# zhihu/rucene

Measured on AMD Instinct MI355X. Metric: queries/sec + postings decoded/sec, BM25 10M-doc synthetic, higher is better.
Workload: dtype u32 decode + f32 BM25

## Files before the change

rucene_amd/csrc/kernels/search_term.hpp:

```cpp
#pragma once
#include "search.hpp"

namespace rgpu {

#ifdef RGPU_EXP_COUNT
__device__ unsigned long long g_term_dbg[4];
#endif

#ifndef RGPU_TERM_PRUNE
#define RGPU_TERM_PRUNE 1
#endif
#ifndef RGPU_TERM_ORDER
#define RGPU_TERM_ORDER 1
#endif
#ifndef RGPU_TERM_EXCHANGE
#define RGPU_TERM_EXCHANGE 2
#endif
#ifndef RGPU_TERM_EXCHANGE_MAX_ITEMS
#define RGPU_TERM_EXCHANGE_MAX_ITEMS 16
#endif
#ifndef RGPU_TERM_WAIT
#define RGPU_TERM_WAIT 0
#endif
#ifndef RGPU_TERM_WAIT_POLLS
// ... 42 lines not shown
  const uint64_t v = __hip_atomic_load(g.keys + (k - 1), __ATOMIC_RELAXED, __HIP_MEMORY_SCOPE_WORKGROUP);
  return ((uint64_t)(uint32_t)readfirstlane((int)(uint32_t)(v >> 32)) << 32) | (uint32_t)readfirstlane((int)(uint32_t)v);
}
#ifndef RGPU_TERM_RANK_MERGE
#define RGPU_TERM_RANK_MERGE 0
#endif
#ifndef RGPU_TERM_RANK_MERGE_MAX
#define RGPU_TERM_RANK_MERGE_MAX 16
#endif
#ifndef RGPU_TERM_LEVEL_CUT
#define RGPU_TERM_LEVEL_CUT 1
#endif
#ifndef RGPU_TERM_LEVEL_CUT_MIN
#define RGPU_TERM_LEVEL_CUT_MIN 16
#endif
#ifdef RGPU_TERM_TRACE
#define TERM_LK_PARAM , uint32_t (&lk)[4]
#define TERM_LK_NOW(v) const uint64_t v = (uint64_t)clock64()
#define TERM_LK_ADD(i, since) lk[i] += (uint32_t)((uint64_t)clock64() - (since))
#define TERM_LK_COUNT(i, n) lk[i] += (uint32_t)(n)
#define TERM_LK_DECL uint32_t lk[4] = {0, 0, 0, 0}
#define TERM_LK_PASS , lk
#else
#define TERM_LK_PARAM
#define TERM_LK_DECL do {} while (0)
#define TERM_LK_PASS
#define TERM_LK_NOW(v) do {} while (0)
#define TERM_LK_ADD(i, since) do {} while (0)
#define TERM_LK_COUNT(i, n) do {} while (0)
#endif
static_assert(RGPU_TERM_RANK_MERGE_MAX >= 3 && RGPU_TERM_RANK_MERGE_MAX <= 64 && 8 * RGPU_TERM_RANK_MERGE_MAX <= TERM_BLOCK_SLAB,
              "the candidates of a rank merge fit one register and the staging slab");
template <bool WIDE>
__device__ __forceinline__ void group_offer2(const GroupList& g, uint64_t key0, uint64_t key1, uint64_t& tau, int k, int lane,
                                             uint64_t floor, uint8_t* slab TERM_LK_PARAM) {
#if RGPU_TERM_LEVEL_CUT
  if (!WIDE && __popcll(__ballot(key0 > tau)) + __popcll(__ballot(key1 > tau)) > (k > RGPU_TERM_LEVEL_CUT_MIN ? k : RGPU_TERM_LEVEL_CUT_MIN)) {
    uint32_t level = 0xffffffffu;
    for (int have = 0; have < k;) {
      const uint32_t h0 = (uint32_t)(key0 >> 32), h1 = (uint32_t)(key1 >> 32);
      const uint32_t b0 = h0 < level ? h0 : 0u, b1 = h1 < level ? h1 : 0u;
      const uint32_t t = wave_reduce_max_u32(b0 > b1 ? b0 : b1);
      if (t == 0u) { level = 0u; break; }
      have += __popcll(__ballot(h0 == t)) + __popcll(__ballot(h1 == t));
      level = t;
    }
    key0 = (uint32_t)(key0 >> 32) >= level ? key0 : 0ull;
    key1 = (uint32_t)(key1 >> 32) >= level ? key1 : 0ull;
  }
#endif
  TERM_LK_NOW(lk_t0);
  TERM_LK_COUNT(2, 1);
  group_lock(g.lock, lane);
  TERM_LK_ADD(0, lk_t0);
  TERM_LK_NOW(lk_t1);
  WaveTopK top;
  top.a = g.keys[lane];
  if (WIDE) top.b = g.keys[64 + lane];
  const uint64_t kth = topk_threshold<WIDE>(top, k);
  tau = kth > floor ? kth : floor;
#if RGPU_TERM_RANK_MERGE
  const uint64_t m0 = __ballot(key0 > tau), m1 = __ballot(key1 > tau);
  const int n0 = __popcll(m0), n = n0 + __popcll(m1);
  TERM_LK_COUNT(3, n);
  if (!WIDE && n > 2 && n <= RGPU_TERM_RANK_MERGE_MAX) {
    uint64_t* stage = reinterpret_cast<uint64_t*>(slab);
    int ln = lane;
    asm volatile("" : "+v"(ln));
    if ((m0 >> ln) & 1ull) stage[mbcnt(m0)] = key0;
    if ((m1 >> ln) & 1ull) stage[n0 + mbcnt(m1)] = key1;
    wave_sync();
    const uint64_t c = ln < n ? stage[ln] : 0ull;
    wave_sync();
    const uint64_t L = top.a;
    int shift = 0;
    for (int i = 0; i < n; ++i) {
      const uint64_t x = readlane64(c, i);
      const bool above = L > x;
      const int at = __popcll(__ballot(above)) + __popcll(__ballot(c > x));
      shift += above ? 0 : 1;
      if (ln == i && at < 64) g.keys[at] = c;
    }
    if (ln + shift < 64) g.keys[ln + shift] = L;
// ... 569 lines not shown
```

rucene_amd/csrc/kernels/search_term_query.hpp:

```cpp
#pragma once
#include "search_term.hpp"

namespace rgpu {

#ifndef RGPU_TERMQ_CAP
#define RGPU_TERMQ_CAP 256
#endif
constexpr int TQ_CAP = RGPU_TERMQ_CAP;
constexpr int TQ_CHUNK_UNROLL = 4;
#ifndef RGPU_TERMQ_STEP_CHUNKS
#define RGPU_TERMQ_STEP_CHUNKS 2
#endif
constexpr int TQ_STEP_CHUNKS = RGPU_TERMQ_STEP_CHUNKS;
#ifndef RGPU_TERMQ_FAST_WAVES
#define RGPU_TERMQ_FAST_WAVES RGPU_TERM_FAST_WAVES
#endif
static_assert(TQ_CAP >= 64 && TQ_CAP <= 65536, "queue positions are u16 and a chunk must fit an empty queue");

__device__ __forceinline__ uint32_t term_thr_of(uint64_t t, int32_t lo) {
  const uint32_t thi = (uint32_t)(t >> 32);
  if (!(thi & 0x80000000u)) return 0u;
  const uint32_t bits = thi & 0x7fffffffu;
  return key_doc(t) <= lo + 1 ? bits + 1u : bits;
}
__device__ __forceinline__ uint32_t term_bound_of(const float* cache, uint64_t w) {
  const uint32_t fmax = (uint32_t)w & 15u;
  uint32_t bb = 0u;
#pragma unroll
  for (int f = 1; f <= SCORE_TABLE_FREQS; ++f) {
    const uint32_t r = (uint32_t)(w >> (4 + 6 * (f - 1))) & 63u;
    const uint32_t sc = __float_as_uint(table_score(cache, r, (uint32_t)f));
    bb = ((uint32_t)f <= fmax && sc > bb) ? sc : bb;
  }
  return fmax > (uint32_t)SCORE_TABLE_FREQS ? 0xffffffffu : bb;
}

#ifdef RGPU_TERM_TRACE
struct TermQueryTraceRec {
  unsigned long long t0, t1;
  int32_t q, nblocks, rounds, entries, unpacked, offers, entered;
  unsigned int d[7];
  unsigned int waves, wave0_cycles;
  unsigned int cyc[8][3];
  unsigned int pad[16];
};
static_assert(sizeof(TermQueryTraceRec) == 3 * sizeof(TermTraceRec), "a workgroup's record takes three slots of g_term_trace");
#define TQ_TR(slot, dep) do { asm volatile("" :: "v"(dep)); tq_d[slot] = (unsigned int)((unsigned long long)wall_clock64() - tq_t0); } while (0)
#else
#define TQ_TR(slot, dep) do {} while (0)
#endif

template <bool LEGACY, bool WIDE, int W>
__global__ __launch_bounds__(64 * W, (LEGACY || WIDE) ? RGPU_TERM_OTHER_WAVES : RGPU_TERMQ_FAST_WAVES)
void k_search_term_query(SegView seg, const DevQuery* __restrict__ queries, const DevTerm* __restrict__ terms,
                         const int32_t* __restrict__ order, int n_queries, int k, unsigned long long* __restrict__ work_slots,
                         const int32_t* __restrict__ qmap, HitOut* __restrict__ hits, int64_t* __restrict__ totals, int32_t doc_base,
                         const TermLaunch* __restrict__ launch) {
  constexpr int LIST_N = WIDE ? 128 : 64;
  constexpr int NT = 64 * W;
  constexpr int DEPTH = PREFETCH_DEPTH;
  __shared__ __attribute__((aligned(16))) uint8_t slabs[W][TERM_BLOCK_SLAB];
  __shared__ float cache[WAVE_CACHE_FLOATS];
  __shared__ uint64_t list[LIST_N];
  __shared__ uint32_t lock_word;
  __shared__ uint32_t e_blk[TQ_CAP], e_row[TQ_CAP], e_bound[TQ_CAP];
  __shared__ int32_t e_lo[TQ_CAP];
  __shared__ uint16_t e_hdr[TQ_CAP], e_order[TQ_CAP];
  __shared__ uint32_t cq[TQ_CHUNK_UNROLL * NT];
  __shared__ uint32_t cnt[TQ_CHUNK_UNROLL * NT / 64 > W * TQ_STEP_CHUNKS ? TQ_CHUNK_UNROLL * NT / 64 : W * TQ_STEP_CHUNKS];
  __shared__ uint32_t cursor;
  __shared__ uint32_t sums[3];
  __shared__ uint64_t floor_s;

  const int lane = lane_id();
  const int wave = wave_id();
  const int tid = (int)threadIdx.x;
#ifdef RGPU_TERM_TRACE
  __shared__ uint32_t tq_w[8][5];
  const unsigned long long tq_t0 = (unsigned long long)wall_clock64();
  const uint64_t tq_c0 = (uint64_t)clock64();
  unsigned int tq_d[7] = {0, 0, 0, 0, 0, 0, 0};
  uint32_t tq_step = 0;
  int tq_rounds = 0, tq_entries = 0;
#endif
  TERM_LK_DECL;
  int q, row, rec;
  if (launch != nullptr) {
    if ((int)blockIdx.x >= n_queries) return;
    const TermLaunch L = launch[blockIdx.x];
    q = row = L.row;
    rec = L.rec;
  } else {
    q = order != nullptr ? order[blockIdx.x] : (int)blockIdx.x;
    if (q >= n_queries) return;
    row = qmap ? qmap[q] : q;
    const DevQuery Q = queries[q];
    rec = Q.n_terms < 1 ? -1 : Q.first_term;
  }
  HitOut* out = hits + (size_t)row * (size_t)k;
  if (rec < 0) {
    if (wave == 0) {
      if (lane < k) out[lane] = HitOut{-1, 0.f};
      if (WIDE && lane + 64 < k) out[lane + 64] = HitOut{-1, 0.f};
      if (lane == 0) {
        totals[row] = 0;
        if (work_slots != nullptr) { work_slots[q] = 0ull; work_slots[n_queries + q] = 0ull; }
      }
    }
    return;
  }
  const DevTerm T = terms[rec];
  TQ_TR(0, T.df);
  const bool has_norms = seg.norms != nullptr;
  const bool tabled = has_norms && seg.n_norm_ranks > 0;
  const bool fast = tabled && seg.live == nullptr && T.weight >= 0.0f && RGPU_TERM_PRUNE && (T.flags & TERM_FLAG_MONOTONE) != 0u;
  const float k1 = seg.sim_tables[(size_t)T.sim_table * 257 + 256];
  const float wk = T.weight * (k1 + 1.0f);
  const uint8_t* term_rows = seg.bstore + T.bs_base;
  const GroupList group{list, &lock_word};
  const int n_chunks = (T.nblocks + 63) >> 6;
  const uint32_t sum_base = (T.dir_base + 63u) >> 6;

  for (int i = tid; i < LIST_N; i += NT) list[i] = 0ull;
  if (tid == 0) { lock_word = 0u; sums[0] = sums[1] = sums[2] = 0u; floor_s = 0ull; cursor = 0u; }
  uint32_t looked = 0, touched = 0;
  int count = 0;
  if (wave == 0) {
    float k1_;
    load_sim_table(seg, T.sim_table, cache, lane, k1_);
    if (tabled) build_score_table(cache, wk, lane);
    TQ_TR(1, cache[lane]);
    if (fast && T.sketch != 0u && seg.sketch != nullptr && k <= TERM_SKETCH_K) {
      const uint64_t f = sketch_floor<WIDE>(seg.sketch + (size_t)(T.sketch - 1u) * TERM_SKETCH_K, cache, k, lane);
      if (lane == 0) floor_s = f;
      touched += 2u * (uint32_t)k;
    }
  }
  __syncthreads();
  const uint64_t floor = ((uint64_t)(uint32_t)readfirstlane((int)(uint32_t)(floor_s >> 32)) << 32) | (uint32_t)readfirstlane((int)(uint32_t)floor_s);
  auto tau_now = [&]() -> uint64_t {
    const uint64_t kth = group_kth<WIDE>(group, k);
    return kth > floor ? kth : floor;
  };
  uint64_t tau = floor;
  TQ_TR(2, (uint32_t)floor);

  if (fast) {
    count = wave == 0 ? 128 * T.nblocks : 0;
    const uint8_t* pn = seg.pnorm + T.pn_base;
    uint8_t* slab = slabs[wave];
    int cnext = 0;
    while (cnext < n_chunks) {
      int nq = 0;
      while (cnext < n_chunks) {
        tau = tau_now();
        uint64_t pass_m[TQ_CHUNK_UNROLL];
        uint32_t tb = 0u;
#pragma unroll
        for (int u = 0; u < TQ_CHUNK_UNROLL; ++u) {
          const int c = cnext + u * NT + tid;
          const bool in = c < n_chunks;
          const bool whole = in && 64 * c + 64 <= T.nblocks;
          const bool worded = whole && seg.dir_sum != nullptr;
          const uint64_t w = worded ? seg.dir_sum[sum_base + (uint32_t)c] : 15ull;
          const int32_t lo = (in && c > 0) ? seg.dir_last[T.dir_base + 64u * (uint32_t)c - 1u] : -1;
          tb += (worded ? 8u : 0u) + ((in && c > 0) ? 4u : 0u);
          pass_m[u] = __ballot(in && term_bound_of(cache, w) >= term_thr_of(tau, lo));
        }
        touched += (uint32_t)wave_reduce_add((int)tb);
#pragma unroll
        for (int u = 0; u < TQ_CHUNK_UNROLL; ++u)
          if (lane == 0) cnt[u * W + wave] = (uint32_t)__popcll(pass_m[u]);
        __syncthreads();
        {
          const int nc = TQ_CHUNK_UNROLL * W;
          const int v = lane < nc ? (int)cnt[lane] : 0;
          const int incl = wave_incl_scan(v);
#pragma unroll
          for (int u = 0; u < TQ_CHUNK_UNROLL; ++u) {
            const int at = readlane(incl - v, u * W + wave);
            if ((pass_m[u] >> lane) & 1ull) cq[at + mbcnt(pass_m[u])] = (uint32_t)(cnext + u * NT + tid);
          }
        }
        const int n_cq = (int)readfirstlane(wave_reduce_add(lane < TQ_CHUNK_UNROLL * W ? (int)cnt[lane] : 0));
        const int window_end = min(n_chunks, cnext + TQ_CHUNK_UNROLL * NT);
        __syncthreads();
        int pos = 0;
        bool full = false;
        while (pos < n_cq) {
          uint64_t bm[TQ_STEP_CHUNKS];
          uint32_t rw[TQ_STEP_CHUNKS], hd[TQ_STEP_CHUNKS];
          int32_t lo[TQ_STEP_CHUNKS];
          int ch[TQ_STEP_CHUNKS];
#pragma unroll
          for (int s = 0; s < TQ_STEP_CHUNKS; ++s) {
            const int ci = pos + wave * TQ_STEP_CHUNKS + s;
            ch[s] = ci < n_cq ? (int)cq[ci] : -1;
            const int nb = ch[s] < 0 ? 0 : min(64, T.nblocks - 64 * ch[s]);
            const bool ok = lane < nb;
            const uint32_t b = T.dir_base + 64u * (uint32_t)(ch[s] < 0 ? 0 : ch[s]) + (uint32_t)lane;
            bm[s] = ok ? seg.dir_bmax[b] : 0ull;
            rw[s] = ok ? seg.dir_row[b] : 0u;
            hd[s] = ok ? (uint32_t)seg.dir_hdr[b] : 0u;
            lo[s] = (ok && b > T.dir_base) ? seg.dir_last[b - 1u] : -1;
            touched += 18u * (uint32_t)nb;
          }
          uint64_t pm[TQ_STEP_CHUNKS];
          uint32_t bd[TQ_STEP_CHUNKS];
#pragma unroll
          for (int s = 0; s < TQ_STEP_CHUNKS; ++s) {
            const int nb = ch[s] < 0 ? 0 : min(64, T.nblocks - 64 * ch[s]);
            bd[s] = term_bound_of(cache, bm[s]);
            pm[s] = __ballot(lane < nb && bd[s] >= term_thr_of(tau, lo[s]));
            if (lane == 0) cnt[wave * TQ_STEP_CHUNKS + s] = (uint32_t)__popcll(pm[s]);
          }
          __syncthreads();
          const int ns = W * TQ_STEP_CHUNKS;
          const int v = lane < ns ? (int)cnt[lane] : 0;
          const int incl = wave_incl_scan(v);
          const int cut = __popcll(__ballot(lane < ns && nq + incl <= TQ_CAP));
#pragma unroll
          for (int s = 0; s < TQ_STEP_CHUNKS; ++s) {
            const int i = wave * TQ_STEP_CHUNKS + s;
            if (i < cut && ((pm[s] >> lane) & 1ull)) {
              const int at = nq + readlane(incl - v, i) + mbcnt(pm[s]);
              e_blk[at] = (uint32_t)(64 * ch[s] + lane);
              e_row[at] = rw[s];
              e_hdr[at] = (uint16_t)hd[s];
              e_lo[at] = lo[s];
              e_bound[at] = bd[s];
            }
          }
          nq += cut > 0 ? readlane(incl, cut - 1) : 0;
          pos = min(n_cq, pos + cut);
          __syncthreads();
          if (cut < ns) { full = true; break; }
        }
        if (full && pos < n_cq) { cnext = (int)cq[pos]; break; }
        cnext = window_end;
        if (full) break;
      }
#ifdef RGPU_TERM_TRACE
      if (tq_rounds == 0) TQ_TR(3, nq);
      tq_rounds += 1;
      tq_entries += nq;
#endif
// ... 139 lines not shown
    atomicAdd(&sums[2], touched);
#ifdef RGPU_TERM_TRACE
    if (wave < 8) { tq_w[wave][0] = lk[0]; tq_w[wave][1] = lk[1]; tq_w[wave][2] = tq_step; tq_w[wave][3] = lk[2]; tq_w[wave][4] = lk[3]; }
#endif
  }
  __syncthreads();
  if (wave != 0) return;
#ifdef RGPU_TERM_TRACE
  TQ_TR(5, sums[0]);
  const unsigned int tq_wave0 = (unsigned int)((uint64_t)clock64() - tq_c0);
#endif
  {
    const bool has_live = seg.live != nullptr;
    int tcount = 0;
    auto collect = [&](int32_t d0, int32_t d1, uint32_t f0, uint32_t f1, uint32_t nb0, uint32_t nb1, bool v0, bool v1) {
      if (has_live) {
        v0 = v0 && doc_in_segment(seg, d0) && doc_is_live(seg.live, d0);
        v1 = v1 && doc_in_segment(seg, d1) && doc_is_live(seg.live, d1);
      }
      float s0, s1;
      const uint32_t fmax = f0 > f1 ? f0 : f1;
      if (tabled && !__ballot((v0 || v1) && fmax > (uint32_t)SCORE_TABLE_FREQS)) {
        s0 = table_score(cache, nb0, v0 ? f0 : 1u);
        s1 = table_score(cache, nb1, v1 ? f1 : 1u);
      } else {
        s0 = bm25_score(wk, (float)(int32_t)f0, has_norms ? cache[nb0] : k1);
        s1 = bm25_score(wk, (float)(int32_t)f1, has_norms ? cache[nb1] : k1);
      }
      tcount += __popcll(__ballot(v0)) + __popcll(__ballot(v1));
      const uint64_t key0 = v0 ? make_key(s0, d0) : 0ull, key1 = v1 ? make_key(s1, d1) : 0ull;
      tau = tau_now();
      if (__ballot((key0 > key1 ? key0 : key1) > tau)) group_offer2<WIDE>(group, key0, key1, tau, k, lane, floor, slabs[0] TERM_LK_PASS);
    };
    if (T.df == 1) {
      const bool v0 = lane == 0;
      const uint32_t nb0 = (has_norms && v0) ? norm_at(seg, T.singleton_doc) : 0u;
      collect(T.singleton_doc, 0, (uint32_t)T.singleton_freq, 1u, nb0, 0u, v0, false);
    } else if (T.tail_n > 0) {
      int32_t d0, d1;
      uint32_t f0, f1;
      tail_load(term_rows, seg.dir_row[T.dir_base + T.nblocks], lane, d0, d1, f0, f1);
      const bool v0 = 2 * lane < T.tail_n, v1 = 2 * lane + 1 < T.tail_n;
      const uint32_t nb0 = (has_norms && v0) ? seg.norms[d0] : 0u, nb1 = (has_norms && v1) ? seg.norms[d1] : 0u;
      collect(d0, d1, f0, f1, nb0, nb1, v0, v1);
    }
    wave_sync();
    const uint64_t a = list[lane];
    const uint64_t b = WIDE ? list[64 + lane] : 0ull;
    if (lane < k) out[lane] = a ? HitOut{key_doc(a) + doc_base, key_score(a)} : HitOut{-1, 0.f};
    if (WIDE && lane + 64 < k) out[lane + 64] = b ? HitOut{key_doc(b) + doc_base, key_score(b)} : HitOut{-1, 0.f};
    if (lane == 0) {
      totals[row] = (int64_t)sums[0] + tcount;
      if (work_slots != nullptr) {
        work_slots[q] = (unsigned long long)sums[2];
        work_slots[n_queries + q] = (unsigned long long)sums[1];
      }
    }
#ifdef RGPU_TERM_TRACE
    TQ_TR(6, a);
    if (lane == 0 && 3 * (int)blockIdx.x + 2 < TERM_TRACE_CAP) {
      TermQueryTraceRec r{};
      r.t0 = tq_t0; r.t1 = (unsigned long long)wall_clock64();
      r.q = q; r.nblocks = T.nblocks; r.rounds = tq_rounds; r.entries = tq_entries; r.unpacked = (int32_t)sums[1];
      for (int i = 0; i < 7; ++i) r.d[i] = tq_d[i];
      r.waves = (unsigned int)W; r.wave0_cycles = tq_wave0;
      int offers = 0, entered = 0;
      for (int w = 0; w < (W < 8 ? W : 8); ++w) {
        r.cyc[w][0] = tq_w[w][0]; r.cyc[w][1] = tq_w[w][1]; r.cyc[w][2] = tq_w[w][2] - tq_w[w][0] - tq_w[w][1];
        offers += (int)tq_w[w][3]; entered += (int)tq_w[w][4];
      }
      r.offers = offers + (int)(lk[2] - tq_w[0][3]); r.entered = entered + (int)(lk[3] - tq_w[0][4]);
      reinterpret_cast<TermQueryTraceRec*>(g_term_trace)[blockIdx.x] = r;
    }
#endif
  }
}

}
```

rucene_amd/csrc/rgpu_api.hip:

```cpp
#include <hip/hip_runtime.h>
#include <hip/hip_ext.h>
#include <rccl/rccl.h>

#include <algorithm>
#include <cstdio>
#include <cstring>
#include <functional>
#include <memory>
#include <mutex>
#include <string>
#include <unordered_map>
#include <tuple>
#include <vector>

#include "../../include/rucene_gpu.h"
#include "host/doc_format.hpp"
#include "host/norms_format.hpp"
#include "host/term_dict.hpp"
#include "host/field_infos_format.hpp"
#include "host/segment_infos_format.hpp"
#include "host/compound_format.hpp"
#include "kernels/prepare.hpp"
#include "kernels/search.hpp"
#include "kernels/search_and.hpp"
// ... 165 lines not shown
  bool and_blocks_per_item_auto = false;
  std::mutex mu;
  DevVec<float> sim_tables;
  int n_sim_tables = 0;
  std::vector<uint8_t> sim_monotone;
  int64_t or_wide_redone = 0;
  std::vector<float> sim_k1;
  std::vector<uint8_t> sim_nonneg;
  std::vector<float> sim_cache_min;
  int64_t or_lazy_evals = 0, or_lazy_only = 0;
  size_t bitmap_bytes = 0;
  size_t bitmap_budget = 0;
  size_t prepared_budget = 0;
  struct UniqSlot { int64_t fp; uint32_t stamp; int32_t idx; };
  std::vector<UniqSlot> lazy_uniq;
  uint32_t lazy_stamp = 0;
  Scratch scr[N_SCRATCH];
  Scratch* S = &scr[0];
  int scr_next = 0;
  DevVec<ScoredPosting> d_runs;
  std::vector<std::function<int32_t()>> pending_or;
  bool defer_or = false;
  bool upload_aside = false;
  bool host_time = false;
  bool stage_by_kernel = true;
  bool term_fold = true;
  bool term_query_kernel = true;
  bool term_plan_resident = true;
  bool term_hot = true;
  bool term_slot_event_bound = true;
  rucene::TermArena arena;
  std::vector<void*> arena_spares;
  int term_query_waves = 4;
  int term_min_item_blocks = 64;
  int term_target_items = 3000;
  int term_split = 8;
  bool phrase_mask_compact = true;
  bool memb_only_on = true;
  bool term_sketches = true;
  DevVec<uint32_t> pos_counts;
  DevVec<unsigned long long> pos_tiles;
  DevVec<int32_t> phrase_docs;
  DevVec<uint64_t> phrase_keys;
  DevVec<int64_t> phrase_redo;
  DevVec<unsigned long long> phrase_count;
  DevVec<unsigned long long> count_rows;
  int count_windows_per_item = 0;
  DevVec<int64_t> phrase_or_prefix;
  DevVec<PhraseRunDev> phrase_or_runs;
  DevVec<uint32_t> phrase_or_buckets;
  DevVec<HitOut> host_api_hits;
  DevVec<int64_t> host_api_totals;
  HostPinned host_api_rows;
  int* d_err = nullptr;
  struct Pass { int stride = 0, col0 = 0; const unsigned long long* ceil_in = nullptr; unsigned long long* ceil_out = nullptr; } pass;
  struct CeilSlot { DevVec<unsigned long long> d; hipEvent_t done = nullptr; bool busy = false; } ceil_slots[N_SCRATCH];
  int ceil_next = 0;
  Scratch* last_and = nullptr;
  int last_and_queries = 0;
  Scratch* last_counted = nullptr;
  const unsigned long long* last_counted_words = nullptr;
  int last_counted_op = -1, last_counted_queries = 0;
  int64_t last_counted_dir_blocks = 0;
  int64_t last_counted_loose = 0;
  int64_t last_counted_postings = 0;
  int64_t last_counted_algo_bytes = 0;
// ... 869 lines not shown
  int count = 0;
  if (hipGetDeviceCount(&count) != hipSuccess || count <= 0)
    return fail(RGPU_ERR_RUNTIME, "no HIP device present: this library has no CPU fallback");
  if (device_ordinal < 0 || device_ordinal >= count) return fail(RGPU_ERR_ILLEGAL_ARGUMENT, "device ordinal out of range");
  HIP_TRY(hipSetDevice(device_ordinal));
  hipDeviceProp_t prop;
  HIP_TRY(hipGetDeviceProperties(&prop, device_ordinal));
  if (std::strncmp(prop.gcnArchName, "gfx950", 6) != 0)
    return fail(RGPU_ERR_RUNTIME, std::string("device is ") + prop.gcnArchName + ", kernels are built for gfx950 only");
  if (cfg && (cfg->blocks_per_item < 0 || cfg->blocks_per_item > (1 << 17)))
    return fail(RGPU_ERR_ILLEGAL_ARGUMENT, "blocks_per_item must be 0 (auto) or 1 .. 131072");
  rgpu_ctx* c = new rgpu_ctx();
  c->device = device_ordinal;
  if (cfg) c->cfg = *cfg;
  c->cfg.abi_version = RGPU_ABI_VERSION;
  if (c->cfg.blocks_per_item <= 0) { c->cfg.blocks_per_item = 32; c->blocks_per_item_auto = true; }
  if (c->cfg.and_blocks_per_item <= 0) { c->cfg.and_blocks_per_item = 8; c->and_blocks_per_item_auto = true; }
  c->bitmap_budget = c->cfg.bitmap_budget_mib > 0 ? (size_t)c->cfg.bitmap_budget_mib << 20 : (size_t)prop.totalGlobalMem / 8;
  c->prepared_budget = c->cfg.prepared_budget_mib > 0 ? (size_t)c->cfg.prepared_budget_mib << 20 : 0;
  if (const char* e = std::getenv("RGPU_TERM_SKETCH")) c->term_sketches = std::atoi(e) != 0;
  if (const char* e = std::getenv("RGPU_UPLOAD_ASIDE")) c->upload_aside = std::atoi(e) != 0;
  if (const char* e = std::getenv("RGPU_AND_MEMB_ONLY")) c->memb_only_on = std::atoi(e) != 0;
  if (const char* e = std::getenv("RGPU_PHRASE_MASK_COMPACT")) c->phrase_mask_compact = std::atoi(e) != 0;
  if (const char* e = std::getenv("RGPU_TERM_TARGET_ITEMS")) c->term_target_items = std::max(256, std::atoi(e));
  if (const char* e = std::getenv("RGPU_HOST_TIME")) c->host_time = std::atoi(e) != 0;
  if (const char* e = std::getenv("RGPU_STAGE_COPY")) c->stage_by_kernel = std::strcmp(e, "dma") != 0;
  if (const char* e = std::getenv("RGPU_TERM_FOLD")) c->term_fold = std::atoi(e) != 0;
  if (const char* e = std::getenv("RGPU_TERM_KERNEL")) c->term_query_kernel = std::strcmp(e, "items") != 0;
  if (const char* e = std::getenv("RGPU_TERM_PLAN")) c->term_plan_resident = std::strcmp(e, "staged") != 0;
  if (const char* e = std::getenv("RGPU_TERM_HOT")) c->term_hot = std::atoi(e) != 0;
  if (const char* e = std::getenv("RGPU_SLOT_EVENT")) c->term_slot_event_bound = std::strcmp(e, "record") != 0;
  if (const char* e = std::getenv("RGPU_TERM_ARENA_RECORDS")) c->arena = rucene::TermArena((uint32_t)std::max(1, std::min(1 << 24, std::atoi(e))));
  if (const char* e = std::getenv("RGPU_TERM_QUERY_WAVES")) { const int w = std::atoi(e); c->term_query_waves = w <= 2 ? 2 : w >= 8 ? 8 : 4; }
  if (const char* e = std::getenv("RGPU_TERM_MIN_ITEM_BLOCKS")) c->term_min_item_blocks = std::max(8, std::min(4096, std::atoi(e)));
  if (const char* e = std::getenv("RGPU_TERM_SPLIT")) c->term_split = std::max(1, std::min(64, std::atoi(e)));
  if (const char* e = std::getenv("RGPU_COUNT_WINDOWS_PER_ITEM")) c->count_windows_per_item = std::max(0, std::min(1 << 20, std::atoi(e)));
  if (const char* e = std::getenv("RGPU_COMM_FORCE_GATHER")) { if (std::atoi(e) != 0) c->cfg.comm_force_gather = 1; }
  std::snprintf(c->name, sizeof c->name, "%s (%s)", prop.name, prop.gcnArchName);
  if (hipStreamCreateWithFlags(&c->stream, hipStreamNonBlocking) != hipSuccess ||
      (c->upload_aside && hipStreamCreateWithFlags(&c->upload, hipStreamNonBlocking) != hipSuccess) ||
      hipMalloc(&c->d_err, 4 * sizeof(int)) != hipSuccess) {
    delete c;
    return fail(RGPU_ERR_RUNTIME, "failed to create stream / error word");
  }
  *out_ctx = c;
  return RGPU_OK;
}

extern "C" void rgpu_shutdown(rgpu_ctx* c) {
  if (!c) return;
  (void)hipSetDevice(c->device);
  c->pending_or.clear();
  (void)hipStreamSynchronize(c->stream);
  drain_events(c);
  arena_drop(c, false);
  for (auto e : c->free_events) (void)hipEventDestroy(e);
  c->sim_tables.release(); for (auto& cs : c->ceil_slots) { cs.d.release(); if (cs.done) (void)hipEventDestroy(cs.done); } c->d_runs.release(); c->pos_counts.release(); c->pos_tiles.release(); c->phrase_docs.release(); c->phrase_keys.release(); c->phrase_redo.release(); c->phrase_count.release(); c->count_rows.release(); c->phrase_or_prefix.release(); c->phrase_or_runs.release(); c->phrase_or_buckets.release(); c->host_api_hits.release(); c->host_api_totals.release(); c->host_api_rows.release();
  for (auto& sc : c->scr) sc.release();
  if (c->d_err) (void)hipFree(c->d_err);
  if (c->upload) { (void)hipStreamSynchronize(c->upload); (void)hipStreamDestroy(c->upload); }
  (void)hipStreamDestroy(c->stream);
  delete c;
}

extern "C" int32_t rgpu_device_name(rgpu_ctx* c, char* buf, size_t len) {
  if (!c || !buf || len == 0) return fail(RGPU_ERR_ILLEGAL_ARGUMENT, "bad arguments");
// ... 5112 lines not shown
      ev = e;
    }
    const hipError_t er = hipEventRecord((hipEvent_t)ev, stream);
    if (er != hipSuccess) { A.give_spare_event(ev); HIP_TRY(er); }
    A.note_upload((uint32_t)first_up, (uint32_t)(first_up + n_up), (uint64_t)(uintptr_t)stream, ev);
  }
  unplace.armed = false;
  if (A.pending_uploads() != 0 && lo <= hi) {
    hipError_t ew = hipSuccess;
    A.for_each_wait((uint64_t)(uintptr_t)stream, lo, hi, [&](void* ev) {
      const hipError_t e = hipStreamWaitEvent(stream, (hipEvent_t)ev, 0);
      if (ew == hipSuccess) ew = e;
    });
    HIP_TRY(ew);
  }
  if (laps) laps->lap(4);
  unsigned long long* d_work = reinterpret_cast<unsigned long long*>(c->S->d_stage.p);
  c->last_counted = c->S;
  c->last_counted_words = d_work;
  c->last_counted_op = RGPU_OP_TERM;
  c->last_counted_queries = nq;
  c->last_counted_postings = postings;
  c->last_counted_dir_blocks = total_blocks;
  c->last_counted_loose = loose;
  const bool wide = k > 64;
  const bool legacy = seg->version < 1;
  const bool bound = c->term_slot_event_bound;
  if (bound && !c->S->done) HIP_TRY(hipEventCreateWithFlags(&c->S->done, hipEventDisableTiming));
  {
    TimedLaunch tl(c, stream, stat_slot_once(c, &c->stat_k_search_term, "k_search_term"), postings);
    const SegView sv = seg_view(seg);
    auto go = [&](auto kern, int waves) -> hipError_t {
      if (bound) RGPU_LAUNCH_WITH_STOP(kern, dim3((unsigned)nq), dim3(64 * waves), 0, stream, c->S->done, sv, (const DevQuery*)nullptr, d_arena, (const int32_t*)nullptr,
                                       (int)nq, (int)k, d_work, (const int32_t*)nullptr, hits_dev, totals_dev, (int32_t)seg->doc_base, (const TermLaunch*)hl);
      else RGPU_LAUNCH(kern, dim3((unsigned)nq), dim3(64 * waves), 0, stream, sv, (const DevQuery*)nullptr, d_arena, (const int32_t*)nullptr, nq, (int)k, d_work,
                       (const int32_t*)nullptr, hits_dev, totals_dev, seg->doc_base, (const TermLaunch*)hl);
      return hipSuccess;
    };
    auto pick = [&](auto legacy_c, auto wide_c) -> hipError_t {
      constexpr bool LG = decltype(legacy_c)::value, WD = decltype(wide_c)::value;
      if (c->term_query_waves == 2) return go(k_search_term_query<LG, WD, 2>, 2);
      if (c->term_query_waves == 8) return go(k_search_term_query<LG, WD, 8>, 8);
      return go(k_search_term_query<LG, WD, 4>, 4);
    };
    hipError_t e;
    if (legacy) e = wide ? pick(std::true_type{}, std::true_type{}) : pick(std::true_type{}, std::false_type{});
    else e = wide ? pick(std::false_type{}, std::true_type{}) : pick(std::false_type{}, std::false_type{});
    HIP_TRY(e);
    c->stats[(size_t)stat_slot_once(c, &c->stat_term_query_launches, "term_query_launches")].launches += 1;
  }
  if (laps) laps->lap(5);
  HIP_TRY(launch_status());
  if (bound) c->S->busy = true;
  else HIP_TRY(scratch_mark(c, stream));
  A.slot_marked((int)(c->S - c->scr), (uint64_t)(uintptr_t)stream);
  c->stats[(size_t)stat_slot_once(c, &c->stat_fused_term_batches, "fused_term_batches")].launches += 1;
  if (laps) { laps->lap(6); laps->done(); }
  *taken = true;
  return RGPU_OK;
}
static int32_t term_batch_fast(rgpu_segment* seg, rucene::BatchPlanner* P, int32_t nq, const int64_t* ids, int32_t k, HitOut* hits_dev,
                               int64_t* totals_dev, hipStream_t stream, bool* taken) {
  rgpu_ctx* c = seg->ctx;
  *taken = false;
  static thread_local HostLaps laps;
  const bool timed = c->host_time;
  if (timed) laps.start();
  const int32_t sim_table = P->sim_table();
  if (!P->flat() || k > RGPU_PASS_K || c->prepared_budget != 0 || sim_table < 0 || sim_table >= c->n_sim_tables || seg->dir_used == 0) return RGPU_OK;
// ... 141 lines not shown
    }
    const size_t staged = o_id + (size_t)items * sizeof(int4);
    if (timed) laps.lap(3);
    HIP_TRY(stage_h2d(c, staged, stream));
  }
  if (timed) laps.lap(4);
  if (!per_query) {
    HIP_TRY(c->S->d_partial_keys.reserve((size_t)items * (size_t)k, 0, stream));
    HIP_TRY(c->S->d_partial_counts.reserve((size_t)items, 0, stream));
  }
  unsigned long long* d_tau = reinterpret_cast<unsigned long long*>(c->S->d_stage.p + o_tau);
  unsigned long long* d_work = reinterpret_cast<unsigned long long*>(c->S->d_stage.p + o_w);
  const DevQuery* dq = reinterpret_cast<const DevQuery*>(c->S->d_stage.p + o_q);
  const DevTerm* dt = reinterpret_cast<const DevTerm*>(c->S->d_stage.p + o_t);
  const int64_t* dp = reinterpret_cast<const int64_t*>(c->S->d_stage.p + o_p);
  const int32_t* dm = reinterpret_cast<const int32_t*>(c->S->d_stage.p + o_m);
  c->last_counted = c->S;
  c->last_counted_words = d_work;
  c->last_counted_op = RGPU_OP_TERM;
  c->last_counted_queries = nq;
  c->last_counted_postings = postings;
  c->last_counted_dir_blocks = total_blocks;
  c->last_counted_loose = loose;
  const bool wide = k > 64;
  const bool legacy = seg->version < 1;
  const TermMerge fold = c->term_fold ? TermMerge{reinterpret_cast<unsigned int*>(c->S->d_stage.p + o_done), dp, hits_dev, totals_dev, nullptr, seg->doc_base, 0, 0}
                                      : TermMerge{};
  if (per_query) {
    TimedLaunch tl(c, stream, "k_search_term", postings);
    const SegView sv = seg_view(seg);
    const int32_t* dord = reinterpret_cast<const int32_t*>(c->S->d_stage.p + o_ord);
    auto go = [&](auto kern, int waves) -> hipError_t {
      RGPU_LAUNCH(kern, dim3((unsigned)nq), dim3(64 * waves), 0, stream, sv, dq, dt, dord, nq, (int)k, d_work, dm, hits_dev, totals_dev, seg->doc_base,
                  (const TermLaunch*)nullptr);
      return hipSuccess;
    };
    auto pick = [&](auto legacy_c, auto wide_c) -> hipError_t {
      constexpr bool LG = decltype(legacy_c)::value, WD = decltype(wide_c)::value;
      if (c->term_query_waves == 2) return go(k_search_term_query<LG, WD, 2>, 2);
      if (c->term_query_waves == 8) return go(k_search_term_query<LG, WD, 8>, 8);
      return go(k_search_term_query<LG, WD, 4>, 4);
    };
    hipError_t e;
    if (legacy) e = wide ? pick(std::true_type{}, std::true_type{}) : pick(std::true_type{}, std::false_type{});
    else e = wide ? pick(std::false_type{}, std::true_type{}) : pick(std::false_type{}, std::false_type{});
    HIP_TRY(e);
    c->stats[(size_t)stat_slot(c, "term_query_launches")].launches += 1;
  } else {
    TimedLaunch tl(c, stream, "k_search_term", postings);
    const unsigned grid = wg_count((items + TERM_WAVES - 1) / TERM_WAVES);
    const size_t lds = term_lds_bytes(wide);
    const SegView sv = seg_view(seg);
    auto go = [&](auto kern) -> hipError_t {
      hipError_t e = set_dynamic_lds_once(c, reinterpret_cast<const void*>(kern), lds);
      if (e != hipSuccess) return e;
      RGPU_LAUNCH(kern, dim3(grid), dim3(TERM_THREADS), lds, stream, sv, dq, dt, reinterpret_cast<const int4*>(c->S->d_stage.p + o_id), nq, items,
                         blocks_per_item, (int)k, c->S->d_partial_keys.p, c->S->d_partial_counts.p, d_tau, d_work, (const unsigned long long*)nullptr, dm, fold);
      return hipSuccess;
    };
    hipError_t e;
    if (legacy) e = wide ? go(k_search_term<true, true>) : go(k_search_term<true, false>);
    else e = wide ? go(k_search_term<false, true>) : go(k_search_term<false, false>);
    HIP_TRY(e);
  }
  if (!per_query && !c->term_fold) {
    if (wide) launch_merge<true>(c, stream, nq, k, dp, seg->doc_base, hits_dev, totals_dev, nq, nullptr, nullptr, dm);
    else launch_merge<false>(c, stream, nq, k, dp, seg->doc_base, hits_dev, totals_dev, nq, nullptr, nullptr, dm);
// ... 147 lines not shown
```

Measured before the change: 64.80 million.

## Add lock-free single-chunk path with per-wave private top-k lists for short terms

For pruned term queries whose posting list fits one directory chunk (up to 64 blocks), each wave loads the directory directly and scores its share of blocks. It keeps a private top-k list aliased onto the cq scratch buffer, and the lists are merged at the end instead of going through the shared locked group list and the chunk queue. The tail/singleton postings are scored up front by the last wave. This targets lock contention, the multi-step chunk-queue bookkeeping and block barriers on short terms. The change also raises the default occupancy hint for the 4/8-wave kernel and skips directory work for empty chunk slots in the general path. The cost is a final merge of W sorted lists, and tau is now per wave, so pruning may be weaker.

```diff
diff --git a/rucene_amd/csrc/kernels/search_term.hpp b/rucene_amd/csrc/kernels/search_term.hpp
--- a/rucene_amd/csrc/kernels/search_term.hpp
+++ b/rucene_amd/csrc/kernels/search_term.hpp
@@ -98,8 +98,7 @@
 static_assert(RGPU_TERM_RANK_MERGE_MAX >= 3 && RGPU_TERM_RANK_MERGE_MAX <= 64 && 8 * RGPU_TERM_RANK_MERGE_MAX <= TERM_BLOCK_SLAB,
               "the candidates of a rank merge fit one register and the staging slab");
 template <bool WIDE>
-__device__ __forceinline__ void group_offer2(const GroupList& g, uint64_t key0, uint64_t key1, uint64_t& tau, int k, int lane,
-                                             uint64_t floor, uint8_t* slab TERM_LK_PARAM) {
+__device__ __forceinline__ void term_level_cut(uint64_t& key0, uint64_t& key1, uint64_t tau, int k) {
 #if RGPU_TERM_LEVEL_CUT
   if (!WIDE && __popcll(__ballot(key0 > tau)) + __popcll(__ballot(key1 > tau)) > (k > RGPU_TERM_LEVEL_CUT_MIN ? k : RGPU_TERM_LEVEL_CUT_MIN)) {
     uint32_t level = 0xffffffffu;
@@ -115,6 +114,24 @@
     key1 = (uint32_t)(key1 >> 32) >= level ? key1 : 0ull;
   }
 #endif
+}
+template <bool WIDE>
+__device__ __forceinline__ void wave_offer2(uint64_t* keys, uint64_t key0, uint64_t key1, uint64_t& tau, int k, int lane, uint64_t floor TERM_LK_PARAM) {
+  term_level_cut<WIDE>(key0, key1, tau, k);
+  TERM_LK_COUNT(2, 1);
+  TERM_LK_COUNT(3, __popcll(__ballot(key0 > tau)) + __popcll(__ballot(key1 > tau)));
+  WaveTopK top;
+  top.a = keys[lane];
+  if (WIDE) top.b = keys[64 + lane];
+  topk_offer<WIDE>(top, key0, tau, k, lane, floor);
+  topk_offer<WIDE>(top, key1, tau, k, lane, floor);
+  keys[lane] = top.a;
+  if (WIDE) keys[64 + lane] = top.b;
+}
+template <bool WIDE>
+__device__ __forceinline__ void group_offer2(const GroupList& g, uint64_t key0, uint64_t key1, uint64_t& tau, int k, int lane,
+                                             uint64_t floor, uint8_t* slab TERM_LK_PARAM) {
+  term_level_cut<WIDE>(key0, key1, tau, k);
   TERM_LK_NOW(lk_t0);
   TERM_LK_COUNT(2, 1);
   group_lock(g.lock, lane);
diff --git a/rucene_amd/csrc/kernels/search_term_query.hpp b/rucene_amd/csrc/kernels/search_term_query.hpp
--- a/rucene_amd/csrc/kernels/search_term_query.hpp
+++ b/rucene_amd/csrc/kernels/search_term_query.hpp
@@ -13,7 +13,10 @@
 #endif
 constexpr int TQ_STEP_CHUNKS = RGPU_TERMQ_STEP_CHUNKS;
 #ifndef RGPU_TERMQ_FAST_WAVES
-#define RGPU_TERMQ_FAST_WAVES RGPU_TERM_FAST_WAVES
+#define RGPU_TERMQ_FAST_WAVES 7
+#endif
+#ifndef RGPU_TERMQ_ONE
+#define RGPU_TERMQ_ONE 1
 #endif
 static_assert(TQ_CAP >= 64 && TQ_CAP <= 65536, "queue positions are u16 and a chunk must fit an empty queue");
 
@@ -50,12 +53,27 @@
 #define TQ_TR(slot, dep) do {} while (0)
 #endif
 
+struct OneChunkDir {
+  uint64_t bm = 0ull;
+  uint32_t rw = 0u, hd = 0u;
+  int32_t lo = -1;
+  __device__ __forceinline__ void load(const SegView& seg, const DevTerm& T, int lane) {
+    if (lane < T.nblocks) {
+      const uint32_t b = T.dir_base + (uint32_t)lane;
+      bm = seg.dir_bmax[b];
+      rw = seg.dir_row[b];
+      hd = (uint32_t)seg.dir_hdr[b];
+      if (lane > 0) lo = seg.dir_last[b - 1u];
+    }
+  }
+};
+
 template <bool LEGACY, bool WIDE, int W>
-__global__ __launch_bounds__(64 * W, (LEGACY || WIDE) ? RGPU_TERM_OTHER_WAVES : RGPU_TERMQ_FAST_WAVES)
+__global__ __launch_bounds__(64 * W, (LEGACY || WIDE) ? RGPU_TERM_OTHER_WAVES : W == 2 ? RGPU_TERM_FAST_WAVES : RGPU_TERMQ_FAST_WAVES)
 void k_search_term_query(SegView seg, const DevQuery* __restrict__ queries, const DevTerm* __restrict__ terms,
                          const int32_t* __restrict__ order, int n_queries, int k, unsigned long long* __restrict__ work_slots,
                          const int32_t* __restrict__ qmap, HitOut* __restrict__ hits, int64_t* __restrict__ totals, int32_t doc_base,
-                         const TermLaunch* __restrict__ launch) {
+                         const TermLaunch* __restrict__ launch, int short_blocks) {
   constexpr int LIST_N = WIDE ? 128 : 64;
   constexpr int NT = 64 * W;
   constexpr int DEPTH = PREFETCH_DEPTH;
@@ -66,7 +84,8 @@
   __shared__ uint32_t e_blk[TQ_CAP], e_row[TQ_CAP], e_bound[TQ_CAP];
   __shared__ int32_t e_lo[TQ_CAP];
   __shared__ uint16_t e_hdr[TQ_CAP], e_order[TQ_CAP];
-  __shared__ uint32_t cq[TQ_CHUNK_UNROLL * NT];
+  __shared__ __attribute__((aligned(16))) uint32_t cq[TQ_CHUNK_UNROLL * NT];
+  static_assert(sizeof(uint32_t) * TQ_CHUNK_UNROLL * NT >= sizeof(uint64_t) * W * LIST_N, "W private lists of LIST_N keys alias cq");
   __shared__ uint32_t cnt[TQ_CHUNK_UNROLL * NT / 64 > W * TQ_STEP_CHUNKS ? TQ_CHUNK_UNROLL * NT / 64 : W * TQ_STEP_CHUNKS];
   __shared__ uint32_t cursor;
   __shared__ uint32_t sums[3];
@@ -121,6 +140,9 @@
   const int n_chunks = (T.nblocks + 63) >> 6;
   const uint32_t sum_base = (T.dir_base + 63u) >> 6;
 
+  const bool one = readfirstlane((int)(RGPU_TERMQ_ONE && fast && short_blocks > 0 && T.nblocks <= short_blocks)) != 0;
+  OneChunkDir oc;
+  uint64_t oc_k0 = 0ull, oc_k1 = 0ull;
   for (int i = tid; i < LIST_N; i += NT) list[i] = 0ull;
   if (tid == 0) { lock_word = 0u; sums[0] = sums[1] = sums[2] = 0u; floor_s = 0ull; cursor = 0u; }
   uint32_t looked = 0, touched = 0;
@@ -129,11 +151,33 @@
     float k1_;
     load_sim_table(seg, T.sim_table, cache, lane, k1_);
     if (tabled) build_score_table(cache, wk, lane);
+    if (one) oc.load(seg, T, lane);
     TQ_TR(1, cache[lane]);
     if (fast && T.sketch != 0u && seg.sketch != nullptr && k <= TERM_SKETCH_K) {
       const uint64_t f = sketch_floor<WIDE>(seg.sketch + (size_t)(T.sketch - 1u) * TERM_SKETCH_K, cache, k, lane);
       if (lane == 0) floor_s = f;
       touched += 2u * (uint32_t)k;
+    }
+  } else if (one) {
+    oc.load(seg, T, lane);
+    if (wave == W - 1 && (T.df == 1 || T.tail_n > 0)) {
+      int32_t d0 = T.singleton_doc, d1 = 0;
+      uint32_t f0 = (uint32_t)T.singleton_freq, f1 = 1u, n0, n1 = 0u;
+      bool v0 = lane == 0, v1 = false;
+      if (T.df == 1) {
+        n0 = v0 ? norm_at(seg, T.singleton_doc) : 0u;
+      } else {
+        tail_load(term_rows, seg.dir_row[T.dir_base + T.nblocks], lane, d0, d1, f0, f1);
+        v0 = 2 * lane < T.tail_n;
+        v1 = 2 * lane + 1 < T.tail_n;
+        n0 = v0 ? seg.norms[d0] : 0u;
+        n1 = v1 ? seg.norms[d1] : 0u;
+      }
+      const float* sim = seg.sim_tables + (size_t)T.sim_table * 257;
+      const float c0 = sim[seg.rank_to_norm[n0]], c1 = sim[seg.rank_to_norm[n1]];
+      const float s0 = bm25_score(wk, (float)(int32_t)f0, c0), s1 = bm25_score(wk, (float)(int32_t)f1, c1);
+      oc_k0 = v0 ? make_key(s0, d0) : 0ull;
+      oc_k1 = v1 ? make_key(s1, d1) : 0ull;
     }
   }
   __syncthreads();
@@ -145,7 +189,115 @@
   uint64_t tau = floor;
   TQ_TR(2, (uint32_t)floor);
 
-  if (fast) {
+  if (one) {
+    const uint8_t* pn = seg.pnorm + T.pn_base;
+    uint8_t* slab = slabs[wave];
+    uint64_t* mine = reinterpret_cast<uint64_t*>(cq) + wave * LIST_N;
+    mine[lane] = 0ull;
+    if (WIDE) mine[64 + lane] = 0ull;
+    if (wave == 0) {
+      count = 128 * T.nblocks;
+      touched += 18u * (uint32_t)T.nblocks;
+    }
+    if (wave == W - 1) {
+      count += T.df == 1 ? 1 : T.tail_n;
+      if (__ballot((oc_k0 > oc_k1 ? oc_k0 : oc_k1) > tau)) wave_offer2<WIDE>(mine, oc_k0, oc_k1, tau, k, lane, floor TERM_LK_PASS);
+    }
+    const uint32_t bd = term_bound_of(cache, oc.bm);
+    const uint64_t pm = __ballot(lane < T.nblocks && bd >= term_thr_of(floor, oc.lo));
+    uint64_t todo = __ballot(((pm >> lane) & 1ull) != 0ull && (mbcnt(pm) & (W - 1)) == wave && bd >= term_thr_of(tau, oc.lo));
+    const int first = todo ? (int)__builtin_ctzll(todo) : 0;
+    if ((todo >> lane) & 1ull) { e_row[lane] = oc.rw; e_hdr[lane] = (uint16_t)oc.hd; e_lo[lane] = oc.lo; e_bound[lane] = bd; }
+    wave_sync();
+#ifdef RGPU_TERM_TRACE
+    tq_entries = __popcll(pm);
+    TQ_TR(3, bd);
+    tq_d[4] = tq_d[3];
+#endif
+    auto take = [&]() -> int {
+      if (!todo) return -1;
+      const int i = (int)__builtin_ctzll(todo);
+      todo &= todo - 1ull;
+      return i;
+    };
+    auto rows_of = [&](int i) -> uint4 { return block_rows_load(block_rows_at(term_rows, e_row[i]), e_hdr[i], lane); };
+    auto norms_of = [&](int i) -> uint32_t {
+      return *reinterpret_cast<const uint16_t*>(pn + (128u * (uint32_t)i + 2u * (uint32_t)lane));
+    };
+    int slot[DEPTH];
+    uint4 ring[DEPTH];
+    uint32_t nring[DEPTH];
+#pragma unroll
+    for (int j = 0; j < DEPTH; ++j) { slot[j] = -1; ring[j] = uint4{0u, 0u, 0u, 0u}; nring[j] = 0u; }
+    if (todo != 0ull) {
+#pragma unroll
+      for (int j = 0; j < DEPTH; ++j) {
+        slot[j] = take();
+        const int pj = slot[j] < 0 ? first : slot[j];
+        ring[j] = rows_of(pj);
+        nring[j] = norms_of(pj);
+      }
+    }
+    auto step = [&](int i, const uint4& rows, uint32_t nn) {
+      const uint32_t hdr = (uint32_t)e_hdr[i];
+      const int32_t lo = e_lo[i];
+      touched += encoded_block_bytes(hdr) + 128u;
+      if (e_bound[i] < term_thr_of(tau, lo)) return;
+      const int bf = hdr_bfreq(hdr);
+      stage_rows(rows, slab, lane);
+      wave_sync();
+      uint32_t f0, f1;
+      bool in_table = true;
+      if (bf) {
+        extract_pair<LEGACY>(slab + SLAB_STREAM, bf, lane, f0, f1);
+        if (bf > 3) in_table = !__ballot((f0 > f1 ? f0 : f1) > (uint32_t)SCORE_TABLE_FREQS);
+      } else {
+        const uint32_t f = (uint32_t)readlane((int)rows.x, 32);
+        f0 = f1 = f;
+        in_table = f <= (uint32_t)SCORE_TABLE_FREQS;
+      }
+      const uint32_t nb0 = nn & 0xffu, nb1 = nn >> 8;
+      float s0, s1;
+      if (in_table) {
+        s0 = table_score(cache, nb0, f0);
+        s1 = table_score(cache, nb1, f1);
+      } else {
+        s0 = bm25_score(wk, (float)(int32_t)f0, cache[nb0]);
+        s1 = bm25_score(wk, (float)(int32_t)f1, cache[nb1]);
+      }
+      looked += 1u;
+      const uint32_t thr = term_thr_of(tau, lo);
+      const uint32_t r0 = __float_as_uint(s0), r1 = __float_as_uint(s1);
+      if (__ballot((r0 > r1 ? r0 : r1) >= thr)) {
+        uint32_t e0, e1;
+        staged_doc_deltas<LEGACY>(slab, rows, hdr, lane, e0, e1);
+        int32_t d0, d1;
+        deltas_to_docs(e0, e1, lo < 0 ? 0 : lo, d0, d1);
+        const uint64_t key0 = make_key(s0, d0), key1 = make_key(s1, d1);
+        if (__ballot((key0 > key1 ? key0 : key1) > tau)) wave_offer2<WIDE>(mine, key0, key1, tau, k, lane, floor TERM_LK_PASS);
+      }
+      wave_sync();
+    };
+    while (slot[0] >= 0) {
+#pragma unroll
+      for (int j = 0; j < DEPTH; ++j) {
+        const uint4 rows = ring[j];
+        const uint32_t nn = nring[j];
+        const int i = slot[j];
+        slot[j] = i >= 0 ? take() : -1;
+        const int pj = slot[j] < 0 ? first : slot[j];
+        ring[j] = rows_of(pj);
+        nring[j] = norms_of(pj);
+        if (i >= 0) {
+          TERM_LK_NOW(tq_s0);
+          step(i, rows, nn);
+#ifdef RGPU_TERM_TRACE
+          tq_step += (uint32_t)((uint64_t)clock64() - tq_s0);
+#endif
+        }
+      }
+    }
+  } else if (fast) {
     count = wave == 0 ? 128 * T.nblocks : 0;
     const uint8_t* pn = seg.pnorm + T.pn_base;
     uint8_t* slab = slabs[wave];
@@ -158,6 +310,7 @@
         uint32_t tb = 0u;
 #pragma unroll
         for (int u = 0; u < TQ_CHUNK_UNROLL; ++u) {
+          if (cnext + u * NT + 64 * wave >= n_chunks) { pass_m[u] = 0ull; continue; }
           const int c = cnext + u * NT + tid;
           const bool in = c < n_chunks;
           const bool whole = in && 64 * c + 64 <= T.nblocks;
@@ -196,9 +349,10 @@
           for (int s = 0; s < TQ_STEP_CHUNKS; ++s) {
             const int ci = pos + wave * TQ_STEP_CHUNKS + s;
             ch[s] = ci < n_cq ? (int)cq[ci] : -1;
-            const int nb = ch[s] < 0 ? 0 : min(64, T.nblocks - 64 * ch[s]);
+            if (ch[s] < 0) { bm[s] = 0ull; rw[s] = 0u; hd[s] = 0u; lo[s] = -1; continue; }
+            const int nb = min(64, T.nblocks - 64 * ch[s]);
             const bool ok = lane < nb;
-            const uint32_t b = T.dir_base + 64u * (uint32_t)(ch[s] < 0 ? 0 : ch[s]) + (uint32_t)lane;
+            const uint32_t b = T.dir_base + 64u * (uint32_t)ch[s] + (uint32_t)lane;
             bm[s] = ok ? seg.dir_bmax[b] : 0ull;
             rw[s] = ok ? seg.dir_row[b] : 0u;
             hd[s] = ok ? (uint32_t)seg.dir_hdr[b] : 0u;
@@ -209,9 +363,14 @@
           uint32_t bd[TQ_STEP_CHUNKS];
 #pragma unroll
           for (int s = 0; s < TQ_STEP_CHUNKS; ++s) {
-            const int nb = ch[s] < 0 ? 0 : min(64, T.nblocks - 64 * ch[s]);
-            bd[s] = term_bound_of(cache, bm[s]);
-            pm[s] = __ballot(lane < nb && bd[s] >= term_thr_of(tau, lo[s]));
+            if (ch[s] < 0) {
+              bd[s] = 0u;
+              pm[s] = 0ull;
+            } else {
+              const int nb = min(64, T.nblocks - 64 * ch[s]);
+              bd[s] = term_bound_of(cache, bm[s]);
+              pm[s] = __ballot(lane < nb && bd[s] >= term_thr_of(tau, lo[s]));
+            }
             if (lane == 0) cnt[wave * TQ_STEP_CHUNKS + s] = (uint32_t)__popcll(pm[s]);
           }
           __syncthreads();
@@ -417,7 +576,14 @@
       tau = tau_now();
       if (__ballot((key0 > key1 ? key0 : key1) > tau)) group_offer2<WIDE>(group, key0, key1, tau, k, lane, floor, slabs[0] TERM_LK_PASS);
     };
-    if (T.df == 1) {
+    WaveTopK merged;
+    if (one) {
+      const uint64_t* wl = reinterpret_cast<const uint64_t*>(cq);
+      merged.a = wl[lane];
+      if (WIDE) merged.b = wl[64 + lane];
+#pragma unroll
+      for (int w = 1; w < W; ++w) topk_merge_sorted<WIDE>(merged, wl[w * LIST_N + lane], WIDE ? wl[w * LIST_N + 64 + lane] : 0ull, lane);
+    } else if (T.df == 1) {
       const bool v0 = lane == 0;
       const uint32_t nb0 = (has_norms && v0) ? norm_at(seg, T.singleton_doc) : 0u;
       collect(T.singleton_doc, 0, (uint32_t)T.singleton_freq, 1u, nb0, 0u, v0, false);
@@ -430,8 +596,8 @@
       collect(d0, d1, f0, f1, nb0, nb1, v0, v1);
     }
     wave_sync();
-    const uint64_t a = list[lane];
-    const uint64_t b = WIDE ? list[64 + lane] : 0ull;
+    const uint64_t a = one ? merged.a : list[lane];
+    const uint64_t b = !WIDE ? 0ull : one ? merged.b : list[64 + lane];
     if (lane < k) out[lane] = a ? HitOut{key_doc(a) + doc_base, key_score(a)} : HitOut{-1, 0.f};
     if (WIDE && lane + 64 < k) out[lane + 64] = b ? HitOut{key_doc(b) + doc_base, key_score(b)} : HitOut{-1, 0.f};
     if (lane == 0) {
@@ -449,6 +615,7 @@
       r.q = q; r.nblocks = T.nblocks; r.rounds = tq_rounds; r.entries = tq_entries; r.unpacked = (int32_t)sums[1];
       for (int i = 0; i < 7; ++i) r.d[i] = tq_d[i];
       r.waves = (unsigned int)W; r.wave0_cycles = tq_wave0;
+      r.pad[0] = one ? 1u : 0u;
       int offers = 0, entered = 0;
       for (int w = 0; w < (W < 8 ? W : 8); ++w) {
         r.cyc[w][0] = tq_w[w][0]; r.cyc[w][1] = tq_w[w][1]; r.cyc[w][2] = tq_w[w][2] - tq_w[w][0] - tq_w[w][1];
diff --git a/rucene_amd/csrc/rgpu_api.hip b/rucene_amd/csrc/rgpu_api.hip
--- a/rucene_amd/csrc/rgpu_api.hip
+++ b/rucene_amd/csrc/rgpu_api.hip
@@ -221,6 +221,7 @@
   rucene::TermArena arena;
   std::vector<void*> arena_spares;
   int term_query_waves = 4;
+  int term_short_blocks = 64;
   int term_min_item_blocks = 64;
   int term_target_items = 3000;
   int term_split = 8;
@@ -1156,6 +1157,7 @@
   if (const char* e = std::getenv("RGPU_SLOT_EVENT")) c->term_slot_event_bound = std::strcmp(e, "record") != 0;
   if (const char* e = std::getenv("RGPU_TERM_ARENA_RECORDS")) c->arena = rucene::TermArena((uint32_t)std::max(1, std::min(1 << 24, std::atoi(e))));
   if (const char* e = std::getenv("RGPU_TERM_QUERY_WAVES")) { const int w = std::atoi(e); c->term_query_waves = w <= 2 ? 2 : w >= 8 ? 8 : 4; }
+  if (const char* e = std::getenv("RGPU_TERM_SHORT_BLOCKS")) c->term_short_blocks = std::max(0, std::min(64, std::atoi(e)));
   if (const char* e = std::getenv("RGPU_TERM_MIN_ITEM_BLOCKS")) c->term_min_item_blocks = std::max(8, std::min(4096, std::atoi(e)));
   if (const char* e = std::getenv("RGPU_TERM_SPLIT")) c->term_split = std::max(1, std::min(64, std::atoi(e)));
   if (const char* e = std::getenv("RGPU_COUNT_WINDOWS_PER_ITEM")) c->count_windows_per_item = std::max(0, std::min(1 << 20, std::atoi(e)));
@@ -6334,9 +6336,10 @@
     const SegView sv = seg_view(seg);
     auto go = [&](auto kern, int waves) -> hipError_t {
       if (bound) RGPU_LAUNCH_WITH_STOP(kern, dim3((unsigned)nq), dim3(64 * waves), 0, stream, c->S->done, sv, (const DevQuery*)nullptr, d_arena, (const int32_t*)nullptr,
-                                       (int)nq, (int)k, d_work, (const int32_t*)nullptr, hits_dev, totals_dev, (int32_t)seg->doc_base, (const TermLaunch*)hl);
+                                       (int)nq, (int)k, d_work, (const int32_t*)nullptr, hits_dev, totals_dev, (int32_t)seg->doc_base, (const TermLaunch*)hl,
+                                       (int)c->term_short_blocks);
       else RGPU_LAUNCH(kern, dim3((unsigned)nq), dim3(64 * waves), 0, stream, sv, (const DevQuery*)nullptr, d_arena, (const int32_t*)nullptr, nq, (int)k, d_work,
-                       (const int32_t*)nullptr, hits_dev, totals_dev, seg->doc_base, (const TermLaunch*)hl);
+                       (const int32_t*)nullptr, hits_dev, totals_dev, seg->doc_base, (const TermLaunch*)hl, c->term_short_blocks);
       return hipSuccess;
     };
     auto pick = [&](auto legacy_c, auto wide_c) -> hipError_t {
@@ -6544,7 +6547,7 @@
     const int32_t* dord = reinterpret_cast<const int32_t*>(c->S->d_stage.p + o_ord);
     auto go = [&](auto kern, int waves) -> hipError_t {
       RGPU_LAUNCH(kern, dim3((unsigned)nq), dim3(64 * waves), 0, stream, sv, dq, dt, dord, nq, (int)k, d_work, dm, hits_dev, totals_dev, seg->doc_base,
-                  (const TermLaunch*)nullptr);
+                  (const TermLaunch*)nullptr, c->term_short_blocks);
       return hipSuccess;
     };
     auto pick = [&](auto legacy_c, auto wide_c) -> hipError_t {
```

Result: faster. 69.31 million (median of 6 runs) (+7.0%).
